# omerbt/TokenFlow

Hardware: NVIDIA H100
Metric: frames/sec for 40-frame 512x512 SD1.5 50-step edit (higher is better)
Workload: dtype fp16

## Files before the change

tokenflow_b200/_build.py:

```python
from __future__ import annotations

import hashlib
import os
import shutil
import subprocess
import sys
from pathlib import Path

PKG_DIR = Path(__file__).resolve().parent
CSRC = PKG_DIR / "csrc"
LIB_PATH = PKG_DIR / "libtokenflow_b200.so"
STAMP = PKG_DIR / ".libtokenflow_b200.stamp"

SOURCES = ["tf_capi.cu", "tf_unit_rows.cu", "tf_propagate.cu", "tf_nn_field.cu", "tf_ext_attn.cu", "tf_cfg_ddim.cu",
           "tf_comm.cu", "tf_body.cu", "tf_pixels.cu", "tf_resize.cu",
           "tf_canny.cu"]
HEADERS = ["tf_common.cuh", "tf_kernels.h", "tf_wgmma.cuh", "../../include/tokenflow_b200.h",
           "../../include/tokenflow_b200_vpred.h"]

NVCC_FLAGS = [
    "-gencode", "arch=compute_90a,code=sm_90a",
    "-O3", "-std=c++17", "-lineinfo",
    "-Xcompiler", "-fPIC",
    "-Xcompiler", "-ffp-contract=off",
    "-Xptxas", "-v",
    "--expt-relaxed-constexpr",
    "-cudart", "static",
]


def _nvcc() -> str:
    for cand in (os.environ.get("NVCC"), shutil.which("nvcc"), "/usr/local/cuda/bin/nvcc"):
        if cand and os.path.exists(cand):
            return cand
    raise RuntimeError("nvcc not found (set NVCC=/path/to/nvcc)")


def _digest() -> str:
    h = hashlib.sha256()
    for name in SOURCES + HEADERS:
        h.update((CSRC / name).read_bytes())
    h.update(" ".join(NVCC_FLAGS).encode())
    return h.hexdigest()


def needs_build() -> bool:
    return not (LIB_PATH.exists() and STAMP.exists() and STAMP.read_text().strip() == _digest())


def build(force: bool = False, verbose: bool = False) -> Path:
    if not force and not needs_build():
# ... 33 lines not shown
```

tokenflow_b200/csrc/tf_body.cu:

```cuda
#include "tf_common.cuh"
#include "tf_kernels.h"

namespace tf {
namespace {

constexpr int kGnMaxThreads = 512;
static_assert(kGnMaxChannels / 8 <= kGnMaxThreads, "one row of 8-channel columns must fit in a CTA");
constexpr int kGnStatsChunkBytes = 64 << 10;
constexpr int kGnApplyChunkBytes = 128 << 10;
constexpr int kGnUnroll = 4;

struct GnLayout {
  int cols, rows, threads;
  long long stats_px, apply_px;
  int stats_chunks, apply_chunks;
};

GnLayout gn_layout(long long hw, int c) {
  GnLayout L;
  L.cols = c / 8;
  L.rows = kGnMaxThreads / L.cols > 0 ? kGnMaxThreads / L.cols : 1;
  L.threads = (L.cols * L.rows + 31) / 32 * 32;
  auto chunk = [&](int bytes) {
    long long px = bytes / (2LL * c);
    px = (px + L.rows - 1) / L.rows * L.rows;
    return px < L.rows ? (long long)L.rows : px;
  };
  L.stats_px = chunk(kGnStatsChunkBytes);
  L.apply_px = chunk(kGnApplyChunkBytes);
  L.stats_chunks = (int)((hw + L.stats_px - 1) / L.stats_px);
  L.apply_chunks = (int)((hw + L.apply_px - 1) / L.apply_px);
  return L;
}

constexpr int kGnG4ApplyChunksPerSample = 64;

GnLayout gn_layout_g4(long long hw, int c) {
  GnLayout L = gn_layout(hw, c);
  long long px = (hw + kGnG4ApplyChunksPerSample - 1) / kGnG4ApplyChunksPerSample;
  px = (px + L.rows - 1) / L.rows * L.rows;
  if (px > L.apply_px) {
    L.apply_px = px;
    L.apply_chunks = (int)((hw + px - 1) / px);
  }
  return L;
}

__device__ __forceinline__ void unpack8(const uint4& raw, float (&v)[8]) {
  const __half2* h = reinterpret_cast<const __half2*>(&raw);
#pragma unroll
  for (int e = 0; e < 4; ++e) {
    const float2 f = __half22float2(h[e]);
    v[2 * e] = f.x;
    v[2 * e + 1] = f.y;
  }
}

__device__ __forceinline__ float round_h(float x) { return __half2float(__float2half_rn(x)); }

template <bool kBias>
__device__ __forceinline__ float group_shift(const __half* xn, const __half* bias_n, int g, int cpg) {
  const int c = g * cpg;
  const float v = __half2float(xn[c]);
  return kBias ? round_h(v + __half2float(bias_n[c])) : v;
}

template <bool kBias, int kCpg>
__global__ void __launch_bounds__(kGnMaxThreads, 2)
gn_stats_kernel(const __half* __restrict__ x, const __half* __restrict__ bias, long long bias_stride, long long hw,
                int C, int cpg_rt, int G, int rows, long long chunk_px, int chunks, double2* __restrict__ ws) {
  const int cpg = kCpg ? kCpg : cpg_rt;
  extern __shared__ double2 part[];
  const int cols = C >> 3;
  const int tid = threadIdx.x;
  const int row = tid / cols, col = tid - row * cols;
  const int n = blockIdx.y, chunk = blockIdx.x;
  const __half* xn = x + (long long)n * hw * C;
  const __half* bias_n = kBias ? bias + (long long)n * bias_stride : nullptr;
  if (row < rows) {
    const int c0 = col * 8;
    float bv[8], shift[8];
    if (kBias) unpack8(*reinterpret_cast<const uint4*>(bias_n + c0), bv);
#pragma unroll
    for (int e = 0; e < 8; ++e) shift[e] = group_shift<kBias>(xn, bias_n, (c0 + e) / cpg, cpg);
    const int g_lo = c0 / cpg;
    int hi_mask = 0;
#pragma unroll
    for (int e = 0; e < 8; ++e) hi_mask |= ((c0 + e) / cpg != g_lo) << e;
    double2 lo = make_double2(0.0, 0.0), hi = make_double2(0.0, 0.0);
    const long long p_begin = (long long)chunk * chunk_px;
    const long long p_end = p_begin + chunk_px < hw ? p_begin + chunk_px : hw;
// ... 114 lines not shown
  for (long long p = p_begin + row; p < p_end; p += (long long)rows * kUnroll) {
    uint4 raw[kUnroll];
#pragma unroll
    for (int u = 0; u < kUnroll; ++u) {
      const long long q = p + (long long)u * rows;
      if (q < p_end) raw[u] = *reinterpret_cast<const uint4*>(xn + q * C + c0);
    }
#pragma unroll
    for (int u = 0; u < kUnroll; ++u) {
      const long long q = p + (long long)u * rows;
      if (q < p_end) {
        float v[8];
        unpack8(raw[u], v);
        uint4 w;
        __half2* h = reinterpret_cast<__half2*>(&w);
#pragma unroll
        for (int e = 0; e < 4; ++e) {
          float y[2];
#pragma unroll
          for (int k = 0; k < 2; ++k) {
            const int i = 2 * e + k;
            const float xv = kBias ? round_h(v[i] + bv[i]) : v[i];
            y[k] = round_h(fmaf(a[i], xv, b[i]));
            if (kSilu) y[k] = y[k] / (1.0f + expf(-y[k]));
          }
          h[e] = __floats2half2_rn(y[0], y[1]);
        }
        *reinterpret_cast<uint4*>(on + q * C + c0) = w;
      }
    }
  }
}

__device__ __forceinline__ float gelu_erf(float v) {
  constexpr float kAlpha = 0.70710678118654752440f;
  return v * 0.5f * (1.0f + erff(v * kAlpha));
}

__device__ __forceinline__ float geglu1(float xv, float gv) { return xv * round_h(gelu_erf(gv)); }

__global__ void __launch_bounds__(256)
geglu_kernel(const __half* __restrict__ xh, const __half* __restrict__ gate, long long n_vec, long long n,
             __half* __restrict__ out) {
  const long long stride = (long long)gridDim.x * blockDim.x;
  for (long long i = (long long)blockIdx.x * blockDim.x + threadIdx.x; i < n_vec; i += stride) {
    float xv[8], gv[8];
    unpack8(reinterpret_cast<const uint4*>(xh)[i], xv);
    unpack8(reinterpret_cast<const uint4*>(gate)[i], gv);
    uint4 w;
    __half2* h = reinterpret_cast<__half2*>(&w);
#pragma unroll
    for (int e = 0; e < 4; ++e) h[e] = __floats2half2_rn(geglu1(xv[2 * e], gv[2 * e]), geglu1(xv[2 * e + 1], gv[2 * e + 1]));
    reinterpret_cast<uint4*>(out)[i] = w;
  }
  if (blockIdx.x == 0 && threadIdx.x == 0) {
    for (long long j = n_vec * 8; j < n; ++j)
      out[j] = __float2half_rn(geglu1(__half2float(xh[j]), __half2float(gate[j])));
  }
}

}

long long group_norm_nhwc_workspace(long long n, long long hw, int c, int groups) {
  if (n <= 0 || hw <= 0 || c <= 0 || (c & 7) || groups <= 0 || c % groups) return 0;
  return n * groups * (long long)gn_layout(hw, c).stats_chunks * (long long)sizeof(double2);
}

namespace {

template <int kCpg>
int launch_gn(const GnLayout& L, const __half* xp, const __half* bp, long long bias_stride, const __half* gp,
              const __half* btp, long long n, long long hw, int c, int groups, float eps, int silu, double2* ws,
              __half* op, cudaStream_t stream, const char* stats_what, const char* apply_what) {
// ... 67 lines not shown
```

tokenflow_b200/csrc/tf_capi.cu:

```cuda
#include <algorithm>
#include <atomic>
#include <cmath>
#include <cstdarg>
#include <cstdio>
#include <cstring>
#include <vector>

#include "../../include/tokenflow_b200.h"
#include "../../include/tokenflow_b200_vpred.h"
#include "tf_common.cuh"
#include "tf_kernels.h"

namespace tf {

static thread_local char g_err[512] = "";
static std::atomic<long long> g_launches{0};

void set_last_error(const char* fmt, ...) {
  va_list ap;
  va_start(ap, fmt);
  vsnprintf(g_err, sizeof(g_err), fmt, ap);
  va_end(ap);
}

int check_cuda(cudaError_t e, const char* what) {
  if (e == cudaSuccess) return TF_OK;
  set_last_error("%s: %s (%s)", what, cudaGetErrorName(e), cudaGetErrorString(e));
  return TF_ERR_CUDA;
}

int sm_count() {
  static int cached[64] = {0};
  int dev = 0;
  if (cudaGetDevice(&dev) != cudaSuccess || dev < 0 || dev >= 64) return 132;
  if (cached[dev] == 0) {
    int n = 0;
    if (cudaDeviceGetAttribute(&n, cudaDevAttrMultiProcessorCount, dev) != cudaSuccess || n <= 0) n = 132;
    cached[dev] = n;
  }
  return cached[dev];
}

// ... 322 lines not shown
  if (!canny_sizes_ok(n, h, w, "tf_canny_u8")) return TF_ERR_INVALID_ARGUMENT;
  if (!(low == low) || !(high == high)) {
    set_last_error("tf_canny_u8: NaN threshold");
    return TF_ERR_INVALID_ARGUMENT;
  }
  if (low > high) std::swap(low, high);
  const double lo = std::floor(low), hi = std::floor(high);
  const int ilo = (int)std::min(std::max(lo, -1.0), 2040.0), ihi = (int)std::min(std::max(hi, -1.0), 2040.0);
  if (n == 0) return TF_OK;
  const long long need = canny_workspace(n, h, w);
  if (workspace_bytes < need) {
    set_last_error("tf_canny_u8: workspace of %lld bytes, %lld needed", (long long)workspace_bytes, need);
    return TF_ERR_INVALID_ARGUMENT;
  }
  if (!frames || !workspace || (!edges_u8 && !cond_f16) || !aligned16(workspace) ||
      (cond_f16 && (reinterpret_cast<uintptr_t>(cond_f16) & 1u))) {
    set_last_error("tf_canny_u8: NULL or misaligned pointer (frames, a 16-byte aligned workspace, and at least one "
                   "output are needed)");
    return TF_ERR_INVALID_ARGUMENT;
  }
  int e = launch_canny(frames, n, h, w, ilo, ihi, workspace, edges_u8, cond_f16, static_cast<cudaStream_t>(stream));
  if (!e) g_launches += 5;
  return e;
}

int tf_geglu(const void* xh, const void* gate, int64_t n, void* out, tf_stream_t stream) {
  if (n < 0) { set_last_error("tf_geglu: n=%lld", (long long)n); return TF_ERR_INVALID_ARGUMENT; }
  if (n == 0) return TF_OK;
  if (!xh || !gate || !out || !aligned16(xh) || !aligned16(gate) || !aligned16(out)) {
    set_last_error("tf_geglu: NULL or misaligned pointer");
    return TF_ERR_INVALID_ARGUMENT;
  }
  int e = launch_geglu(xh, gate, n, out, static_cast<cudaStream_t>(stream));
  if (!e) g_launches += 1;
  return e;
}

int tf_nn_field(const void* x_unit, const void* piv_unit, const int32_t* kf_a, const int32_t* kf_b, int F, int S,
                int dim, int K, int32_t* idx_a, int32_t* idx_b, tf_stream_t stream) {
  if (F < 0 || S < 0 || dim <= 0 || (dim & 7) || K <= 0) {
    set_last_error("tf_nn_field: bad shape F=%d S=%d dim=%d K=%d", F, S, dim, K);
    return TF_ERR_INVALID_ARGUMENT;
  }
  if (F > 0 && !kf_a) { set_last_error("tf_nn_field: kf_a is NULL"); return TF_ERR_INVALID_ARGUMENT; }
  for (int f0 = 0; f0 < F; f0 += kMaxFrames) {
    FrameTable tab;
    const int fc = F - f0 < kMaxFrames ? F - f0 : kMaxFrames;
    if (int e = fill_table(tab, kf_a + f0, kf_b ? kf_b + f0 : nullptr, nullptr, fc, K, "tf_nn_field")) return e;
  }
  if (F == 0 || S == 0) return TF_OK;
  bool need_b = false;
  if (kf_b) for (int f = 0; f < F; ++f) need_b |= kf_b[f] >= 0;
  if (!x_unit || !piv_unit || !idx_a || (need_b && !idx_b) || !aligned16(x_unit) || !aligned16(piv_unit)) {
    set_last_error("tf_nn_field: NULL or misaligned pointer");
    return TF_ERR_INVALID_ARGUMENT;
  }
  const __half* xu = static_cast<const __half*>(x_unit);
  for (int f0 = 0; f0 < F; f0 += kMaxFrames) {
    FrameTable tab;
    const int fc = F - f0 < kMaxFrames ? F - f0 : kMaxFrames;
    fill_table(tab, kf_a + f0, kf_b ? kf_b + f0 : nullptr, nullptr, fc, K, "tf_nn_field");
    const long long off = (long long)f0 * S;
    int e = launch_nn_field(xu + off * dim, piv_unit, tab, fc, S, dim, K, idx_a + off, idx_b ? idx_b + off : nullptr,
                            static_cast<cudaStream_t>(stream));
    if (e) return e;
    g_launches += 1;
// ... 166 lines not shown
```

tokenflow_b200/csrc/tf_common.cuh:

```cuda
#pragma once

#include <cuda.h>
#include <cuda_fp16.h>
#include <cuda_runtime.h>
#include <stdint.h>
#include <stdio.h>

namespace tf {

void set_last_error(const char* fmt, ...);
int  check_cuda(cudaError_t e, const char* what);

enum Status : int {
  TF_OK = 0,
  TF_ERR_INVALID_ARGUMENT = 1,
  TF_ERR_CUDA = 2,
  TF_ERR_UNSUPPORTED = 3,
  TF_ERR_DRIVER = 4,
};

CUresult encode_tiled(CUtensorMap* map, CUtensorMapDataType dtype, uint32_t rank, const void* base,
                      const uint64_t* dims, const uint64_t* strides_bytes ,
                      const uint32_t* box, CUtensorMapSwizzle swizzle);

// ... 19 lines not shown
               : "memory");
}
__device__ __forceinline__ bool mbar_try_wait(uint64_t* bar, uint32_t parity) {
  uint32_t ok;
  asm volatile(
      "{\n\t.reg .pred p;\n\t"
      "mbarrier.try_wait.parity.shared::cta.b64 p, [%1], %2;\n\t"
      "selp.u32 %0, 1, 0, p;\n\t}\n"
      : "=r"(ok)
      : "r"(smem_u32(bar)), "r"(parity)
      : "memory");
  return ok != 0;
}
__device__ __forceinline__ uint64_t global_timer_ns() {
  uint64_t t;
  asm volatile("mov.u64 %0, %%globaltimer;" : "=l"(t));
  return t;
}
__device__ __forceinline__ void mbar_wait(uint64_t* bar, uint32_t parity) {
  uint32_t spins = 0;
  uint64_t t0 = 0;
  while (!mbar_try_wait(bar, parity)) {
    if ((++spins & 2047u) == 0) {
      const uint64_t now = global_timer_ns();
      if (t0 == 0) t0 = now;
      if (now - t0 > 2000000000ull) __trap();
    }
  }
}

__device__ __forceinline__ void tma_prefetch_desc(const CUtensorMap* m) {
  asm volatile("prefetch.tensormap [%0];" ::"l"(reinterpret_cast<uint64_t>(m)) : "memory");
}
__device__ __forceinline__ void tma_load_3d(void* smem_dst, const CUtensorMap* m, uint64_t* bar, int c0,
                                            int c1, int c2) {
  asm volatile(
      "cp.async.bulk.tensor.3d.shared::cluster.global.tile.mbarrier::complete_tx::bytes"
      " [%0], [%1, {%3, %4, %5}], [%2];"
      ::"r"(smem_u32(smem_dst)), "l"(reinterpret_cast<uint64_t>(m)), "r"(smem_u32(bar)), "r"(c0), "r"(c1),
      "r"(c2)
      : "memory");
}
__device__ __forceinline__ void tma_load_4d(void* smem_dst, const CUtensorMap* m, uint64_t* bar, int c0,
                                            int c1, int c2, int c3) {
  asm volatile(
      "cp.async.bulk.tensor.4d.shared::cluster.global.tile.mbarrier::complete_tx::bytes"
      " [%0], [%1, {%3, %4, %5, %6}], [%2];"
      ::"r"(smem_u32(smem_dst)), "l"(reinterpret_cast<uint64_t>(m)), "r"(smem_u32(bar)), "r"(c0), "r"(c1),
      "r"(c2), "r"(c3)
      : "memory");
}

__device__ __forceinline__ uint64_t wgmma_desc(uint32_t smem_addr, uint32_t lbo_bytes, uint32_t sbo_bytes) {
  uint64_t d = 0;
  d |= static_cast<uint64_t>((smem_addr & 0x3FFFFu) >> 4);
  d |= static_cast<uint64_t>((lbo_bytes >> 4) & 0x3FFFu) << 16;
  d |= static_cast<uint64_t>((sbo_bytes >> 4) & 0x3FFFu) << 32;
  d |= static_cast<uint64_t>(1) << 62;
  return d;
}
__device__ __forceinline__ void wgmma_fence() { asm volatile("wgmma.fence.sync.aligned;" ::: "memory"); }
__device__ __forceinline__ void wgmma_commit() { asm volatile("wgmma.commit_group.sync.aligned;" ::: "memory"); }
template <int kPending>
__device__ __forceinline__ void wgmma_wait() {
  asm volatile("wgmma.wait_group.sync.aligned %0;" ::"n"(kPending) : "memory");
}
template <int N>
__device__ __forceinline__ void reg_fence(float (&r)[N]) {
#pragma unroll
  for (int i = 0; i < N; ++i) asm volatile("" : "+f"(r[i])::"memory");
}

__device__ __forceinline__ uint32_t pack_f16x2_rn(float lo, float hi) {
  uint32_t r;
  asm("cvt.rn.f16x2.f32 %0, %1, %2;" : "=r"(r) : "f"(hi), "f"(lo));
  return r;
}
__device__ __forceinline__ float fast_exp2(float x) {
  float y;
  asm("ex2.approx.ftz.f32 %0, %1;" : "=f"(y) : "f"(x));
  return y;
}
#endif

}
```

tokenflow_b200/csrc/tf_kernels.h:

```cpp
#pragma once

#include <cuda_runtime.h>
#include <stdint.h>

namespace tf {

constexpr int kMaxFrames = 64;
struct FrameTable {
  int32_t kf_a[kMaxFrames];
  int32_t kf_b[kMaxFrames];
  float w[kMaxFrames];
};

int launch_unit_rows(const void* x, int x_is_f32, long long rows, int dim, long long row_stride, void* out_f16,
                     cudaStream_t stream);

int launch_layernorm_unit_rows(const void* x_f16, long long rows, int dim, long long row_stride, const float* gamma,
                               const float* beta, float eps, void* out_f16, cudaStream_t stream);

int launch_layernorm_rows(const void* x_f16, long long rows, int dim, long long row_stride, const float* gamma,
                          const float* beta, float eps, void* y_out, long long y_row_stride, void* unit_out,
                          long long unit_row_stride, long long unit_rows, cudaStream_t stream);

int launch_cfg_ddim(const void* eps_uncond, const void* eps_cond, const void* x, const float* coef_dev, float guidance,
                    long long n, void* out, cudaStream_t stream);
int launch_ddim(const void* eps, const void* x, const float* coef_dev, long long n, void* out, cudaStream_t stream);
int launch_cfg_ddim_v(const void* v_uncond, const void* v_cond, const void* x, const float* coef_dev, float guidance,
                      long long n, void* out, cudaStream_t stream);
int launch_ddim_v(const void* v, const void* x, const float* coef_dev, long long n, void* out, cudaStream_t stream);

constexpr int kGnMaxChannels = 4096;
long long group_norm_nhwc_workspace(long long n, long long hw, int c, int groups);
int launch_group_norm_nhwc(const void* x, const void* bias, long long bias_stride, const void* gamma, const void* beta,
                           long long n, long long hw, int c, int groups, float eps, int silu, void* workspace,
                           void* out, cudaStream_t stream);
int launch_geglu(const void* xh, const void* gate, long long n, void* out, cudaStream_t stream);

int launch_frames_to_nhwc(const void* frames, long long n, void* out, cudaStream_t stream);
int launch_nhwc_to_frames(const void* x, long long n, void* frames, cudaStream_t stream);

int resize_taps(int in, int out);
void resize_coeffs(int in, int out, int32_t* bounds, int32_t* coeffs);
int launch_resize_h(const void* in, long long n_rows, int w_in, int w, const int32_t* bounds, const int32_t* coeffs,
                    int taps, void* out, cudaStream_t stream);
int launch_resize_v(const void* in, long long n, int h_in, int h, int w, const int32_t* bounds, const int32_t* coeffs,
                    int taps, void* out, cudaStream_t stream);

long long canny_workspace(long long n, int h, int w);
int launch_canny(const void* frames, long long n, int h, int w, int low, int high, void* workspace, void* edges,
                 void* cond, cudaStream_t stream);

int launch_propagate(const void* A, const int32_t* idx_a, const int32_t* idx_b, const FrameTable& tab, int F,
                     int S, int dim, int K, const void* residual, void* out, int out_is_f32, long long F_total,
                     cudaStream_t stream);

int launch_nn_field(const void* x_unit, const void* piv_unit, const FrameTable& tab, int F, int S, int dim,
                    int K, int32_t* idx_a, int32_t* idx_b, cudaStream_t stream);

struct AttnSample {
  int32_t out_sample;
  int32_t q_sample;
  int32_t k_sample0;
  int32_t v_sample0;
  int32_t n_kv;
};
constexpr int kMaxAttnSamples = 160;
struct AttnTable {
  AttnSample s[kMaxAttnSamples];
};
// ... 25 lines not shown
```

tokenflow_b200/csrc/tf_pixels.cu:

```cuda
#include "tf_common.cuh"
#include "tf_kernels.h"

namespace tf {
namespace {

__device__ __forceinline__ float round_h(float x) { return __half2float(__float2half_rn(x)); }

__device__ __forceinline__ __half byte_to_input(unsigned v) {
  const float unit = round_h(__fdiv_rn((float)v, 255.0f));
  return __float2half_rn(round_h(2.0f * unit) - 1.0f);
}

__device__ __forceinline__ unsigned char output_to_byte(float x) {
  float y = round_h(round_h(x * 0.5f) + 0.5f);
  if (isnan(y)) return 0;
  y = fminf(fmaxf(y, 0.0f), 1.0f);
  return (unsigned char)round_h(y * 255.0f);
}

__global__ void __launch_bounds__(256) frames_to_input_kernel(const uint8_t* __restrict__ in, long long n_vec,
                                                              long long n, __half* __restrict__ out) {
  const long long stride = (long long)gridDim.x * blockDim.x;
  for (long long i = (long long)blockIdx.x * blockDim.x + threadIdx.x; i < n_vec; i += stride) {
    const uint2 raw = reinterpret_cast<const uint2*>(in)[i];
    uint4 w;
    __half* h = reinterpret_cast<__half*>(&w);
#pragma unroll
    for (int e = 0; e < 8; ++e) h[e] = byte_to_input(((e < 4 ? raw.x : raw.y) >> (8 * (e & 3))) & 0xffu);
    reinterpret_cast<uint4*>(out)[i] = w;
  }
  if (blockIdx.x == 0)
    for (long long j = n_vec * 8 + threadIdx.x; j < n; j += blockDim.x) out[j] = byte_to_input(in[j]);
}

__global__ void __launch_bounds__(256) output_to_frames_kernel(const __half* __restrict__ in, long long n_vec,
                                                               long long n, uint8_t* __restrict__ out) {
  const long long stride = (long long)gridDim.x * blockDim.x;
  for (long long i = (long long)blockIdx.x * blockDim.x + threadIdx.x; i < n_vec; i += stride) {
    const uint4 raw = reinterpret_cast<const uint4*>(in)[i];
// ... 38 lines not shown
```

tokenflow_b200/ops.py:

```python
from __future__ import annotations

import ctypes
from pathlib import Path
from typing import Optional, Sequence, Tuple

import torch

LIB_NAME = "libtokenflow_b200.so"
TF_MAX_FRAMES = 64
TF_MAX_ATTN_SAMPLES = 160
TF_COMM_ID_BYTES = 128

_c_i32p = ctypes.POINTER(ctypes.c_int32)
_c_f32p = ctypes.POINTER(ctypes.c_float)

_SIGNATURES = {
    "tf_version": (ctypes.c_int, []),
    "tf_last_error": (ctypes.c_char_p, []),
    "tf_launch_count": (ctypes.c_int64, []),
    "tf_unit_rows": (ctypes.c_int, [ctypes.c_void_p, ctypes.c_int, ctypes.c_int64, ctypes.c_int, ctypes.c_int64,
                                    ctypes.c_void_p, ctypes.c_void_p]),
    "tf_layernorm_unit_rows": (ctypes.c_int, [ctypes.c_void_p, ctypes.c_int64, ctypes.c_int, ctypes.c_int64,
                                              ctypes.c_void_p, ctypes.c_void_p, ctypes.c_float, ctypes.c_void_p,
                                              ctypes.c_void_p]),
# ... 16 lines not shown
                                    ctypes.c_void_p, ctypes.c_int, ctypes.c_void_p]),
    "tf_ext_attn_fwd": (ctypes.c_int, [ctypes.c_void_p, ctypes.c_void_p, ctypes.c_void_p, ctypes.c_int64,
                                       ctypes.c_int, ctypes.c_int, ctypes.c_int, ctypes.c_int, ctypes.c_float,
                                       ctypes.c_int, ctypes.c_void_p, ctypes.c_void_p]),
    "tf_ext_attn_fwd_rows": (ctypes.c_int, [ctypes.c_void_p, ctypes.c_int, ctypes.c_int64, ctypes.c_void_p,
                                            ctypes.c_void_p, ctypes.c_int, ctypes.c_int64, ctypes.c_int, _c_i32p,
                                            _c_i32p, _c_i32p, _c_i32p, _c_i32p, ctypes.c_int, ctypes.c_int,
                                            ctypes.c_int, ctypes.c_float, ctypes.c_int, ctypes.c_int, ctypes.c_void_p,
                                            ctypes.c_void_p]),
    "tf_group_norm_nhwc_workspace": (ctypes.c_int64, [ctypes.c_int64, ctypes.c_int64, ctypes.c_int, ctypes.c_int]),
    "tf_group_norm_nhwc": (ctypes.c_int, [ctypes.c_void_p, ctypes.c_void_p, ctypes.c_int64, ctypes.c_void_p,
                                          ctypes.c_void_p, ctypes.c_int64, ctypes.c_int64, ctypes.c_int, ctypes.c_int,
                                          ctypes.c_float, ctypes.c_int, ctypes.c_void_p, ctypes.c_int64,
                                          ctypes.c_void_p, ctypes.c_void_p]),
    "tf_frames_to_nhwc": (ctypes.c_int, [ctypes.c_void_p, ctypes.c_int64, ctypes.c_void_p, ctypes.c_void_p]),
    "tf_nhwc_to_frames": (ctypes.c_int, [ctypes.c_void_p, ctypes.c_int64, ctypes.c_void_p, ctypes.c_void_p]),
    "tf_resize_taps": (ctypes.c_int, [ctypes.c_int, ctypes.c_int]),
    "tf_resize_coeffs": (ctypes.c_int, [ctypes.c_int, ctypes.c_int, ctypes.c_void_p, ctypes.c_void_p]),
    "tf_resize_u8": (ctypes.c_int, [ctypes.c_void_p, ctypes.c_int64, ctypes.c_int, ctypes.c_int, ctypes.c_int,
                                    ctypes.c_int, ctypes.c_void_p, ctypes.c_void_p, ctypes.c_int, ctypes.c_void_p,
                                    ctypes.c_void_p, ctypes.c_int, ctypes.c_void_p, ctypes.c_void_p, ctypes.c_void_p]),
    "tf_canny_workspace": (ctypes.c_int64, [ctypes.c_int64, ctypes.c_int, ctypes.c_int]),
    "tf_canny_u8": (ctypes.c_int, [ctypes.c_void_p, ctypes.c_int64, ctypes.c_int, ctypes.c_int, ctypes.c_double,
                                   ctypes.c_double, ctypes.c_void_p, ctypes.c_int64, ctypes.c_void_p, ctypes.c_void_p,
                                   ctypes.c_void_p]),
    "tf_geglu": (ctypes.c_int, [ctypes.c_void_p, ctypes.c_void_p, ctypes.c_int64, ctypes.c_void_p, ctypes.c_void_p]),
}

_VPRED_SIGNATURES = {
    "tf_cfg_ddim_v": _SIGNATURES["tf_cfg_ddim"],
    "tf_ddim_v": _SIGNATURES["tf_ddim"],
}


class TokenflowB200Error(RuntimeError):
    pass


def library_path() -> Path:
    return Path(__file__).resolve().parent / LIB_NAME


_LIB = None


def load_library() -> ctypes.CDLL:
    global _LIB
    if _LIB is not None:
        return _LIB
    path = library_path()
    if not path.exists():
        raise TokenflowB200Error(
            f"{path} is missing: build it with `python -m tokenflow_b200._build` "
            "(or __graft_entry__.build()).  tokenflow_b200 has no fallback path.")
    lib = ctypes.CDLL(str(path))
    for name, (res, args) in list(_SIGNATURES.items()) + list(_VPRED_SIGNATURES.items()):
        fn = getattr(lib, name)
        fn.restype = res
        fn.argtypes = args
    _LIB = lib
    return lib


def exported_symbols() -> Sequence[str]:
    return tuple(_SIGNATURES.keys())


def blend_weights(n_frames: int) -> Sequence[float]:
    f = torch.arange(0, n_frames)
    d1 = torch.abs(f - n_frames // 2)
    d2 = torch.abs(f + n_frames - n_frames // 2)
    return torch.sigmoid(d2 / (d1 + d2)).tolist()


def propagate_bytes(F_: int, S: int, dim: int, kf_a, kf_b, with_residual: bool, out_esz: int = 2) -> float:
    kfs = {int(a) for a in kf_a} | {int(b) for b in kf_b if int(b) >= 0}
    n_idx = F_ + sum(1 for b in kf_b if int(b) >= 0)
    return (3.0 * F_ * S * dim * out_esz + (3.0 * F_ * S * dim * 2 if with_residual else 0.0)
            + 3.0 * len(kfs) * S * dim * 2 + 4.0 * S * n_idx)


def _dense(t: torch.Tensor, memory_format=torch.contiguous_format) -> torch.Tensor:
    if t.is_contiguous(memory_format=memory_format) and t.data_ptr() % 16 == 0:
        return t
    return t.clone(memory_format=memory_format)


def _i32(vals: Sequence[int]):
    return (ctypes.c_int32 * len(vals))(*[int(v) for v in vals])
# ... 364 lines not shown
        assert frames.dtype == torch.uint8 and frames.dim() == 4 and frames.shape[-1] == 3 and frames.is_cuda
        assert edges or cond
        frames = frames.contiguous()
        n, h, w, _ = frames.shape
        dev = frames.device
        ws_bytes = int(self.lib.tf_canny_workspace(n, h, w))
        if ws_bytes < 0:
            self._check(1, "tf_canny_workspace")
        ws = torch.empty(max(ws_bytes, 16), dtype=torch.uint8, device=dev)
        e = c = None
        if edges:
            e = out_edges if out_edges is not None else torch.empty((n, h, w), dtype=torch.uint8, device=dev)
            assert e.shape == (n, h, w) and e.dtype == torch.uint8 and e.is_contiguous()
        if cond:
            c = out_cond if out_cond is not None else torch.empty((n, 3, h, w), dtype=torch.float16, device=dev,
                                                                  memory_format=torch.channels_last)
            assert c.shape == (n, 3, h, w) and c.dtype == torch.float16 and c.is_contiguous(memory_format=torch.channels_last)
        work = 3.0 * n * h * w + (n * h * w if edges else 0) + (6.0 * n * h * w if cond else 0)
        ptr = lambda t: t.data_ptr() if t is not None else None
        self._timed("tf_canny_u8", work, lambda: self._check(self.lib.tf_canny_u8(
            frames.data_ptr(), n, h, w, float(low), float(high), ws.data_ptr(), ws.numel(), ptr(e), ptr(c),
            self._stream()), "tf_canny_u8"))
        return e, c

    def geglu(self, xh: torch.Tensor, gate: torch.Tensor) -> torch.Tensor:
        assert xh.dtype == gate.dtype == torch.float16 and xh.shape == gate.shape
        xh, gate = _dense(xh), _dense(gate)
        out = torch.empty_like(xh)
        n = xh.numel()
        self._timed("tf_geglu", 3.0 * n * 2, lambda: self._check(
            self.lib.tf_geglu(xh.data_ptr(), gate.data_ptr(), n, out.data_ptr(), self._stream()), "tf_geglu"))
        return out


_DEFAULT_OPS = None


def default_ops() -> CudaOps:
    global _DEFAULT_OPS
    if _DEFAULT_OPS is None:
        _DEFAULT_OPS = CudaOps()
    return _DEFAULT_OPS


_BODY_OPS = False


def body_ops() -> Optional[CudaOps]:
    global _BODY_OPS
    if _BODY_OPS is False:
        try:
            _BODY_OPS = default_ops()
        except TokenflowB200Error:
            _BODY_OPS = None
    return _BODY_OPS


def all_gather(t: torch.Tensor, world_size: int, group=None, comm=None) -> torch.Tensor:
    if world_size == 1:
        return t
    if comm is not None and t.is_cuda:
        return comm.all_gather(t)
    import torch.distributed as dist
    t = t.contiguous()
    out = torch.empty((world_size * t.shape[0],) + tuple(t.shape[1:]), dtype=t.dtype, device=t.device)
    dist.all_gather_into_tensor(out, t, group=group)
# ... 42 lines not shown
```

tokenflow_b200/sd_unet.py:

```python
from __future__ import annotations

import math
from dataclasses import dataclass
from typing import Optional, Tuple

import torch
import torch.nn as nn
import torch.nn.functional as F


@dataclass
class UNetConfig:
    in_channels: int = 4
    out_channels: int = 4
    block_out_channels: Tuple[int, ...] = (320, 640, 1280, 1280)
    layers_per_block: int = 2
    cross_attention_dim: int = 768
    num_heads: Tuple[int, ...] = (8, 8, 8, 8)
    norm_num_groups: int = 32
    use_linear_projection: bool = False
    sample_size: int = 64


def sd15_config() -> UNetConfig:
# ... 58 lines not shown
        ctx = cross_attention_dim if cross_attention_dim is not None else query_dim
        self.to_q = nn.Linear(query_dim, inner, bias=False)
        self.to_k = nn.Linear(ctx, inner, bias=False)
        self.to_v = nn.Linear(ctx, inner, bias=False)
        self.to_out = nn.ModuleList([nn.Linear(inner, query_dim), nn.Dropout(0.0)])

    def head_to_batch_dim(self, t: torch.Tensor) -> torch.Tensor:
        b, s, _ = t.shape
        h = self.heads
        return t.reshape(b, s, h, -1).permute(0, 2, 1, 3).reshape(b * h, s, -1)

    def batch_to_head_dim(self, t: torch.Tensor) -> torch.Tensor:
        bh, s, d = t.shape
        h = self.heads
        return t.reshape(bh // h, h, s, d).permute(0, 2, 1, 3).reshape(bh // h, s, d * h)

    def forward(self, hidden_states, encoder_hidden_states=None, attention_mask=None):
        ctx = hidden_states if encoder_hidden_states is None else encoder_hidden_states
        b, s, _ = hidden_states.shape
        h = self.heads
        q = self.to_q(hidden_states).view(b, s, h, -1).transpose(1, 2)
        k = self.to_k(ctx).view(b, ctx.shape[1], h, -1).transpose(1, 2)
        v = self.to_v(ctx).view(b, ctx.shape[1], h, -1).transpose(1, 2)
        o = F.scaled_dot_product_attention(q, k, v, attn_mask=attention_mask, scale=self.scale)
        o = o.transpose(1, 2).reshape(b, s, -1)
        return self.to_out[1](self.to_out[0](o))


class GEGLU(nn.Module):
    def __init__(self, dim_in: int, dim_out: int):
        super().__init__()
        self.proj = nn.Linear(dim_in, dim_out * 2)

    def forward(self, x):
        w_x, w_g = self.proj.weight.chunk(2, dim=0)
        b_x, b_g = self.proj.bias.chunk(2, dim=0)
        xh, g = F.linear(x, w_x, b_x), F.linear(x, w_g, b_g)
        if xh.is_cuda and xh.dtype == g.dtype == torch.float16:
            from .ops import body_ops
            ops = body_ops()
            if ops is not None:
                return ops.geglu(xh, g)
        return xh * F.gelu(g)


class FeedForward(nn.Module):
    def __init__(self, dim: int, mult: int = 4):
        super().__init__()
        self.net = nn.ModuleList([GEGLU(dim, dim * mult), nn.Dropout(0.0), nn.Linear(dim * mult, dim)])

    def forward(self, x):
        for m in self.net:
            x = m(x)
        return x


class BasicTransformerBlock(nn.Module):

    def __init__(self, dim: int, heads: int, dim_head: int, cross_attention_dim: int):
        super().__init__()
        self.only_cross_attention = False
        self.use_ada_layer_norm = False
        self.use_ada_layer_norm_zero = False
        self.norm1 = nn.LayerNorm(dim)
        self.attn1 = Attention(dim, None, heads, dim_head)
        self.norm2 = BodyLayerNorm(dim)
        self.attn2 = Attention(dim, cross_attention_dim, heads, dim_head)
# ... 297 lines not shown
```

Measured before the change: 2.881.

## Fuse GEGLU projection GEMM with bias and gelu gating into one WGMMA kernel

Adds a persistent warp-specialized Hopper GEMM (TMA loads, 4-stage mbarrier pipeline, two consumer warpgroups, WGMMA) that computes both the value and gate halves of the GEGLU projection per tile. It applies bias, gelu and gating in the epilogue and TMA-stores the result. This replaces two separate cuBLAS linears plus an elementwise geglu kernel, removing the round trip of two large intermediate activations through HBM. The trade-off is a hand-written GEMM with a fixed 256x64 tile that may be slower than cuBLAS on the matmul itself, and it keeps an fp16 rounding order meant to match the unfused path.

```diff
diff --git a/include/tokenflow_b200_gemm.h b/include/tokenflow_b200_gemm.h
--- /dev/null
+++ b/include/tokenflow_b200_gemm.h
@@ -0,0 +1,18 @@
+#ifndef TOKENFLOW_B200_GEMM_H_
+#define TOKENFLOW_B200_GEMM_H_
+
+#include <stdint.h>
+
+#include "tokenflow_b200.h"
+
+#ifdef __cplusplus
+extern "C" {
+#endif
+
+int tf_geglu_gemm(const void* x, const void* w, const void* bias, int64_t M, int K, int inner, void* out,
+                  tf_stream_t stream);
+
+#ifdef __cplusplus
+}
+#endif
+#endif
diff --git a/tokenflow_b200/_build.py b/tokenflow_b200/_build.py
--- a/tokenflow_b200/_build.py
+++ b/tokenflow_b200/_build.py
@@ -14,9 +14,9 @@
 
 SOURCES = ["tf_capi.cu", "tf_unit_rows.cu", "tf_propagate.cu", "tf_nn_field.cu", "tf_ext_attn.cu", "tf_cfg_ddim.cu",
            "tf_comm.cu", "tf_body.cu", "tf_pixels.cu", "tf_resize.cu",
-           "tf_canny.cu"]
+           "tf_canny.cu", "tf_geglu_gemm.cu"]
 HEADERS = ["tf_common.cuh", "tf_kernels.h", "tf_wgmma.cuh", "../../include/tokenflow_b200.h",
-           "../../include/tokenflow_b200_vpred.h"]
+           "../../include/tokenflow_b200_vpred.h", "../../include/tokenflow_b200_gemm.h"]
 
 NVCC_FLAGS = [
     "-gencode", "arch=compute_90a,code=sm_90a",
diff --git a/tokenflow_b200/csrc/tf_body.cu b/tokenflow_b200/csrc/tf_body.cu
--- a/tokenflow_b200/csrc/tf_body.cu
+++ b/tokenflow_b200/csrc/tf_body.cu
@@ -55,8 +55,6 @@
     v[2 * e + 1] = f.y;
   }
 }
-
-__device__ __forceinline__ float round_h(float x) { return __half2float(__float2half_rn(x)); }
 
 template <bool kBias>
 __device__ __forceinline__ float group_shift(const __half* xn, const __half* bias_n, int g, int cpg) {
@@ -237,13 +235,6 @@
   }
 }
 
-__device__ __forceinline__ float gelu_erf(float v) {
-  constexpr float kAlpha = 0.70710678118654752440f;
-  return v * 0.5f * (1.0f + erff(v * kAlpha));
-}
-
-__device__ __forceinline__ float geglu1(float xv, float gv) { return xv * round_h(gelu_erf(gv)); }
-
 __global__ void __launch_bounds__(256)
 geglu_kernel(const __half* __restrict__ xh, const __half* __restrict__ gate, long long n_vec, long long n,
              __half* __restrict__ out) {
diff --git a/tokenflow_b200/csrc/tf_capi.cu b/tokenflow_b200/csrc/tf_capi.cu
--- a/tokenflow_b200/csrc/tf_capi.cu
+++ b/tokenflow_b200/csrc/tf_capi.cu
@@ -8,6 +8,7 @@
 
 #include "../../include/tokenflow_b200.h"
 #include "../../include/tokenflow_b200_vpred.h"
+#include "../../include/tokenflow_b200_gemm.h"
 #include "tf_common.cuh"
 #include "tf_kernels.h"
 
@@ -396,6 +397,23 @@
     return TF_ERR_INVALID_ARGUMENT;
   }
   int e = launch_geglu(xh, gate, n, out, static_cast<cudaStream_t>(stream));
+  if (!e) g_launches += 1;
+  return e;
+}
+
+int tf_geglu_gemm(const void* x, const void* w, const void* bias, int64_t M, int K, int inner, void* out,
+                  tf_stream_t stream) {
+  if (M < 0 || M >= INT32_MAX - 128 || K <= 0 || (K & 7) || inner <= 0 || (inner & 7)) {
+    set_last_error("tf_geglu_gemm: bad shape M=%lld K=%d inner=%d (K %% 8 == 0, inner %% 8 == 0, M < 2^31 - 128)",
+                   (long long)M, K, inner);
+    return TF_ERR_INVALID_ARGUMENT;
+  }
+  if (M == 0) return TF_OK;
+  if (!x || !w || !bias || !out || !aligned16(x) || !aligned16(w) || !aligned16(bias) || !aligned16(out)) {
+    set_last_error("tf_geglu_gemm: NULL or misaligned pointer");
+    return TF_ERR_INVALID_ARGUMENT;
+  }
+  int e = launch_geglu_gemm(x, w, bias, M, K, inner, out, static_cast<cudaStream_t>(stream));
   if (!e) g_launches += 1;
   return e;
 }
diff --git a/tokenflow_b200/csrc/tf_common.cuh b/tokenflow_b200/csrc/tf_common.cuh
--- a/tokenflow_b200/csrc/tf_common.cuh
+++ b/tokenflow_b200/csrc/tf_common.cuh
@@ -75,6 +75,13 @@
 __device__ __forceinline__ void tma_prefetch_desc(const CUtensorMap* m) {
   asm volatile("prefetch.tensormap [%0];" ::"l"(reinterpret_cast<uint64_t>(m)) : "memory");
 }
+__device__ __forceinline__ void tma_load_2d(void* smem_dst, const CUtensorMap* m, uint64_t* bar, int c0, int c1) {
+  asm volatile(
+      "cp.async.bulk.tensor.2d.shared::cluster.global.tile.mbarrier::complete_tx::bytes"
+      " [%0], [%1, {%3, %4}], [%2];"
+      ::"r"(smem_u32(smem_dst)), "l"(reinterpret_cast<uint64_t>(m)), "r"(smem_u32(bar)), "r"(c0), "r"(c1)
+      : "memory");
+}
 __device__ __forceinline__ void tma_load_3d(void* smem_dst, const CUtensorMap* m, uint64_t* bar, int c0,
                                             int c1, int c2) {
   asm volatile(
@@ -93,6 +100,19 @@
       "r"(c2), "r"(c3)
       : "memory");
 }
+
+__device__ __forceinline__ void tma_store_2d(const CUtensorMap* m, const void* smem_src, int c0, int c1) {
+  asm volatile("cp.async.bulk.tensor.2d.global.shared::cta.bulk_group [%0, {%2, %3}], [%1];"
+               ::"l"(reinterpret_cast<uint64_t>(m)), "r"(smem_u32(smem_src)), "r"(c0), "r"(c1)
+               : "memory");
+}
+__device__ __forceinline__ void tma_store_commit() { asm volatile("cp.async.bulk.commit_group;" ::: "memory"); }
+__device__ __forceinline__ void tma_store_wait_read() { asm volatile("cp.async.bulk.wait_group.read 0;" ::: "memory"); }
+__device__ __forceinline__ void tma_store_wait_all() { asm volatile("cp.async.bulk.wait_group 0;" ::: "memory"); }
+__device__ __forceinline__ void fence_proxy_async_smem() {
+  asm volatile("fence.proxy.async.shared::cta;" ::: "memory");
+}
+__device__ __forceinline__ void wg_bar_sync(int id) { asm volatile("bar.sync %0, 128;" ::"r"(id) : "memory"); }
 
 __device__ __forceinline__ uint64_t wgmma_desc(uint32_t smem_addr, uint32_t lbo_bytes, uint32_t sbo_bytes) {
   uint64_t d = 0;
@@ -124,6 +144,13 @@
   asm("ex2.approx.ftz.f32 %0, %1;" : "=f"(y) : "f"(x));
   return y;
 }
+__device__ __forceinline__ float round_h(float x) { return __half2float(__float2half_rn(x)); }
+
+__device__ __forceinline__ float gelu_erf(float v) {
+  constexpr float kAlpha = 0.70710678118654752440f;
+  return v * 0.5f * (1.0f + erff(v * kAlpha));
+}
+__device__ __forceinline__ float geglu1(float xv, float gv) { return xv * round_h(gelu_erf(gv)); }
 #endif
 
 }
diff --git a/tokenflow_b200/csrc/tf_geglu_gemm.cu b/tokenflow_b200/csrc/tf_geglu_gemm.cu
--- /dev/null
+++ b/tokenflow_b200/csrc/tf_geglu_gemm.cu
@@ -0,0 +1,188 @@
+#include "tf_common.cuh"
+#include "tf_kernels.h"
+#include "tf_wgmma.cuh"
+
+namespace tf {
+namespace {
+
+constexpr int kConsumers = 2;
+constexpr int kBlockM = 128 * kConsumers;
+constexpr int kBlockN = 64;
+constexpr int kChunkK = 64;
+constexpr int kStages = 4;
+constexpr int kThreads = 128 * kConsumers + 32;
+constexpr int kABytes = kBlockM * 128;
+constexpr int kBHalfBytes = kBlockN * 128;
+constexpr int kStageBytes = kABytes + 2 * kBHalfBytes;
+constexpr int kOutBytes = 128 * kBlockN * 2;
+constexpr size_t kSmemBytes =
+    1024 + (size_t)kStages * kStageBytes + (size_t)kConsumers * kOutBytes + 2 * kStages * sizeof(uint64_t);
+
+__device__ __forceinline__ void stage_half(const float (&acc)[64], const __half* __restrict__ bias, int n0, int inner,
+                                           int r0, int col0, uint8_t* tile) {
+#pragma unroll
+  for (int jb = 0; jb < 8; ++jb) {
+    const int col = n0 + col0 + 8 * jb;
+    float2 bx = make_float2(0.f, 0.f), bg = make_float2(0.f, 0.f);
+    if (col < inner) {
+      bx = __half22float2(*reinterpret_cast<const __half2*>(bias + col));
+      bg = __half22float2(*reinterpret_cast<const __half2*>(bias + inner + col));
+    }
+#pragma unroll
+    for (int r = 0; r < 2; ++r) {
+      const int row = r0 + 8 * r;
+      const float x0 = round_h(acc[4 * jb + 2 * r] + bx.x);
+      const float x1 = round_h(acc[4 * jb + 2 * r + 1] + bx.y);
+      const float g0 = round_h(acc[4 * (jb + 8) + 2 * r] + bg.x);
+      const float g1 = round_h(acc[4 * (jb + 8) + 2 * r + 1] + bg.y);
+      *reinterpret_cast<__half2*>(tile + row * 128 + ((jb ^ (row & 7)) << 4) + col0 * 2) =
+          __floats2half2_rn(geglu1(x0, g0), geglu1(x1, g1));
+    }
+  }
+}
+
+__global__ void __launch_bounds__(kThreads, 1)
+geglu_gemm_kernel(const __grid_constant__ CUtensorMap map_x, const __grid_constant__ CUtensorMap map_w,
+                  const __grid_constant__ CUtensorMap map_out, const __half* __restrict__ bias, int inner,
+                  int n_col_tiles, long long n_tiles, int n_k) {
+  extern __shared__ uint8_t smem_raw[];
+  uint8_t* smem = reinterpret_cast<uint8_t*>((reinterpret_cast<uintptr_t>(smem_raw) + 1023) & ~uintptr_t(1023));
+  uint8_t* out_tiles = smem + kStages * kStageBytes;
+  uint64_t* full = reinterpret_cast<uint64_t*>(out_tiles + kConsumers * kOutBytes);
+  uint64_t* empty = full + kStages;
+
+  if (threadIdx.x == 0) {
+    tma_prefetch_desc(&map_x);
+    tma_prefetch_desc(&map_w);
+    tma_prefetch_desc(&map_out);
+    for (int i = 0; i < kStages; ++i) {
+      mbar_init(&full[i], 1);
+      mbar_init(&empty[i], 4 * kConsumers);
+    }
+    fence_mbar_init();
+  }
+  __syncthreads();
+
+  if (threadIdx.x >= 128 * kConsumers) {
+    if (threadIdx.x == 128 * kConsumers) {
+      int st = 0;
+      uint32_t ph = 0;
+      bool refill = false;
+      for (long long t = blockIdx.x; t < n_tiles; t += gridDim.x) {
+        const int m0 = (int)(t / n_col_tiles) * kBlockM;
+        const int n0 = (int)(t % n_col_tiles) * kBlockN;
+        for (int kc = 0; kc < n_k; ++kc) {
+          if (refill) mbar_wait(&empty[st], ph ^ 1u);
+          uint8_t* dst = smem + st * kStageBytes;
+          mbar_arrive_expect_tx(&full[st], (uint32_t)kStageBytes);
+          tma_load_2d(dst, &map_x, &full[st], kc * kChunkK, m0);
+          tma_load_3d(dst + kABytes, &map_w, &full[st], kc * kChunkK, n0, 0);
+          tma_load_3d(dst + kABytes + kBHalfBytes, &map_w, &full[st], kc * kChunkK, n0, 1);
+          if (++st == kStages) { st = 0; ph ^= 1u; refill = true; }
+        }
+      }
+    }
+    return;
+  }
+
+  const int wg = threadIdx.x >> 7;
+  const int warp = (threadIdx.x >> 5) & 3;
+  const int lane = threadIdx.x & 31;
+  const uint32_t ring = smem_u32(smem);
+  auto release = [&](int s) {
+    __syncwarp();
+    if (lane == 0) mbar_arrive(&empty[s]);
+  };
+  int st = 0, prev = 0;
+  uint32_t ph = 0;
+  for (long long t = blockIdx.x; t < n_tiles; t += gridDim.x) {
+    float acc0[64], acc1[64];
+#pragma unroll
+    for (int i = 0; i < 64; ++i) acc0[i] = acc1[i] = 0.0f;
+    for (int kc = 0; kc < n_k; ++kc) {
+      mbar_wait(&full[st], ph);
+      __syncwarp();
+      const uint32_t b = ring + st * kStageBytes + kABytes;
+      const uint32_t a = ring + st * kStageBytes + wg * 128 * 128;
+      wgmma_fence();
+#pragma unroll
+      for (int k4 = 0; k4 < kChunkK / 16; ++k4) {
+        const uint64_t db = wgmma_desc(b + k4 * 32, 16, 1024);
+        wgmma_ss<128>(acc0, wgmma_desc(a + k4 * 32, 16, 1024), db, 1u);
+        wgmma_ss<128>(acc1, wgmma_desc(a + 64 * 128 + k4 * 32, 16, 1024), db, 1u);
+      }
+      wgmma_commit();
+      if (kc > 0) {
+        wgmma_wait<1>();
+        release(prev);
+      }
+      prev = st;
+      if (++st == kStages) { st = 0; ph ^= 1u; }
+    }
+    wgmma_wait<0>();
+    reg_fence(acc0);
+    reg_fence(acc1);
+    release(prev);
+
+    const int m0 = (int)(t / n_col_tiles) * kBlockM + 128 * wg;
+    const int n0 = (int)(t % n_col_tiles) * kBlockN;
+    uint8_t* tile = out_tiles + wg * kOutBytes;
+    const bool issuer = (threadIdx.x & 127) == 0;
+    if (issuer) tma_store_wait_read();
+    wg_bar_sync(1 + wg);
+    const int r0 = 16 * warp + (lane >> 2);
+    stage_half(acc0, bias, n0, inner, r0, 2 * (lane & 3), tile);
+    stage_half(acc1, bias, n0, inner, r0 + 64, 2 * (lane & 3), tile);
+    fence_proxy_async_smem();
+    wg_bar_sync(1 + wg);
+    if (issuer) {
+      tma_store_2d(&map_out, tile, n0, m0);
+      tma_store_commit();
+    }
+  }
+  if ((threadIdx.x & 127) == 0) tma_store_wait_all();
+}
+
+}
+
+int launch_geglu_gemm(const void* x, const void* w, const void* bias, long long M, int K, int inner, void* out,
+                      cudaStream_t stream) {
+  if (M == 0) return TF_OK;
+  const int n_col_tiles = (inner + kBlockN - 1) / kBlockN;
+  const long long n_tiles = (M + kBlockM - 1) / kBlockM * n_col_tiles;
+  const int n_k = (K + kChunkK - 1) / kChunkK;
+  CUtensorMap map_x, map_w, map_out;
+  {
+    const uint64_t dims[2] = {(uint64_t)K, (uint64_t)M};
+    const uint64_t strides[1] = {(uint64_t)K * 2};
+    const uint32_t box[2] = {(uint32_t)kChunkK, (uint32_t)kBlockM};
+    CUresult r = encode_tiled(&map_x, CU_TENSOR_MAP_DATA_TYPE_FLOAT16, 2, x, dims, strides, box,
+                              CU_TENSOR_MAP_SWIZZLE_128B);
+    if (r != CUDA_SUCCESS) { set_last_error("tf_geglu_gemm: cuTensorMapEncodeTiled(x) failed: %d", (int)r); return TF_ERR_DRIVER; }
+  }
+  {
+    const uint64_t dims[3] = {(uint64_t)K, (uint64_t)inner, 2};
+    const uint64_t strides[2] = {(uint64_t)K * 2, (uint64_t)inner * K * 2};
+    const uint32_t box[3] = {(uint32_t)kChunkK, (uint32_t)kBlockN, 1};
+    CUresult r = encode_tiled(&map_w, CU_TENSOR_MAP_DATA_TYPE_FLOAT16, 3, w, dims, strides, box,
+                              CU_TENSOR_MAP_SWIZZLE_128B);
+    if (r != CUDA_SUCCESS) { set_last_error("tf_geglu_gemm: cuTensorMapEncodeTiled(w) failed: %d", (int)r); return TF_ERR_DRIVER; }
+  }
+  {
+    const uint64_t dims[2] = {(uint64_t)inner, (uint64_t)M};
+    const uint64_t strides[1] = {(uint64_t)inner * 2};
+    const uint32_t box[2] = {(uint32_t)kBlockN, 128};
+    CUresult r = encode_tiled(&map_out, CU_TENSOR_MAP_DATA_TYPE_FLOAT16, 2, out, dims, strides, box,
+                              CU_TENSOR_MAP_SWIZZLE_128B);
+    if (r != CUDA_SUCCESS) { set_last_error("tf_geglu_gemm: cuTensorMapEncodeTiled(out) failed: %d", (int)r); return TF_ERR_DRIVER; }
+  }
+  if (check_cuda(cudaFuncSetAttribute(geglu_gemm_kernel, cudaFuncAttributeMaxDynamicSharedMemorySize, (int)kSmemBytes),
+                 "tf_geglu_gemm smem attribute"))
+    return TF_ERR_CUDA;
+  const long long grid = n_tiles < (long long)sm_count() ? n_tiles : (long long)sm_count();
+  geglu_gemm_kernel<<<(unsigned)grid, kThreads, kSmemBytes, stream>>>(
+      map_x, map_w, map_out, static_cast<const __half*>(bias), inner, n_col_tiles, n_tiles, n_k);
+  return check_cuda(cudaGetLastError(), "tf_geglu_gemm launch");
+}
+
+}
diff --git a/tokenflow_b200/csrc/tf_kernels.h b/tokenflow_b200/csrc/tf_kernels.h
--- a/tokenflow_b200/csrc/tf_kernels.h
+++ b/tokenflow_b200/csrc/tf_kernels.h
@@ -35,6 +35,8 @@
                            long long n, long long hw, int c, int groups, float eps, int silu, void* workspace,
                            void* out, cudaStream_t stream);
 int launch_geglu(const void* xh, const void* gate, long long n, void* out, cudaStream_t stream);
+int launch_geglu_gemm(const void* x, const void* w, const void* bias, long long M, int K, int inner, void* out,
+                      cudaStream_t stream);
 
 int launch_frames_to_nhwc(const void* frames, long long n, void* out, cudaStream_t stream);
 int launch_nhwc_to_frames(const void* x, long long n, void* frames, cudaStream_t stream);
diff --git a/tokenflow_b200/csrc/tf_pixels.cu b/tokenflow_b200/csrc/tf_pixels.cu
--- a/tokenflow_b200/csrc/tf_pixels.cu
+++ b/tokenflow_b200/csrc/tf_pixels.cu
@@ -3,8 +3,6 @@
 
 namespace tf {
 namespace {
-
-__device__ __forceinline__ float round_h(float x) { return __half2float(__float2half_rn(x)); }
 
 __device__ __forceinline__ __half byte_to_input(unsigned v) {
   const float unit = round_h(__fdiv_rn((float)v, 255.0f));
diff --git a/tokenflow_b200/ops.py b/tokenflow_b200/ops.py
--- a/tokenflow_b200/ops.py
+++ b/tokenflow_b200/ops.py
@@ -72,6 +72,11 @@
     "tf_ddim_v": _SIGNATURES["tf_ddim"],
 }
 
+_GEMM_SIGNATURES = {
+    "tf_geglu_gemm": (ctypes.c_int, [ctypes.c_void_p, ctypes.c_void_p, ctypes.c_void_p, ctypes.c_int64, ctypes.c_int,
+                                     ctypes.c_int, ctypes.c_void_p, ctypes.c_void_p]),
+}
+
 
 class TokenflowB200Error(RuntimeError):
     pass
@@ -94,7 +99,8 @@
             f"{path} is missing: build it with `python -m tokenflow_b200._build` "
             "(or __graft_entry__.build()).  tokenflow_b200 has no fallback path.")
     lib = ctypes.CDLL(str(path))
-    for name, (res, args) in list(_SIGNATURES.items()) + list(_VPRED_SIGNATURES.items()):
+    for name, (res, args) in (list(_SIGNATURES.items()) + list(_VPRED_SIGNATURES.items())
+                              + list(_GEMM_SIGNATURES.items())):
         fn = getattr(lib, name)
         fn.restype = res
         fn.argtypes = args
@@ -525,6 +531,31 @@
             self.lib.tf_geglu(xh.data_ptr(), gate.data_ptr(), n, out.data_ptr(), self._stream()), "tf_geglu"))
         return out
 
+    @staticmethod
+    def geglu_proj_supported(x: torch.Tensor, weight: torch.Tensor, bias: Optional[torch.Tensor]) -> bool:
+        if bias is None or not (x.is_cuda and x.dtype == weight.dtype == bias.dtype == torch.float16):
+            return False
+        K = x.shape[-1]
+        if x.dim() < 2 or weight.dim() != 2 or weight.shape[1] != K or weight.shape[0] % 2 or bias.shape != weight.shape[:1]:
+            return False
+        inner = weight.shape[0] // 2
+        return K % 8 == 0 and inner % 8 == 0 and inner > 0 \
+            and x.numel() // K < 2 ** 31 - 128 \
+            and weight.device == bias.device == x.device
+
+    def geglu_proj(self, x: torch.Tensor, weight: torch.Tensor, bias: torch.Tensor) -> torch.Tensor:
+        K = x.shape[-1]
+        inner = weight.shape[0] // 2
+        x2 = _dense(x.reshape(-1, K))
+        w, b = _dense(weight), _dense(bias)
+        M = x2.shape[0]
+        out = torch.empty((M, inner), dtype=torch.float16, device=x.device)
+        nbytes = 2.0 * (M * K + 2 * inner * K + 2 * inner + M * inner)
+        self._timed("tf_geglu", nbytes, lambda: self._check(
+            self.lib.tf_geglu_gemm(x2.data_ptr(), w.data_ptr(), b.data_ptr(), M, K, inner, out.data_ptr(),
+                                   self._stream()), "tf_geglu_gemm"))
+        return out.view(*x.shape[:-1], inner)
+
 
 _DEFAULT_OPS = None
 
diff --git a/tokenflow_b200/sd_unet.py b/tokenflow_b200/sd_unet.py
--- a/tokenflow_b200/sd_unet.py
+++ b/tokenflow_b200/sd_unet.py
@@ -114,7 +114,26 @@
         super().__init__()
         self.proj = nn.Linear(dim_in, dim_out * 2)
 
-    def forward(self, x):
+    def _half_params(self):
+        w, b = self.proj.weight, self.proj.bias
+        key = (w.data_ptr(), w._version, b.data_ptr(), b._version)
+        cache = self.__dict__.get("_tf_half_params")
+        if cache is None or cache[0] != key:
+            cache = (key, w.detach().half().contiguous(), b.detach().half().contiguous())
+            self.__dict__["_tf_half_params"] = cache
+        return cache[1], cache[2]
+
+    def forward(self, x):
+        w, b = self.proj.weight, self.proj.bias
+        if x.is_cuda and x.dtype == torch.float16 and b is not None:
+            if w.dtype != torch.float16 and torch.is_autocast_enabled("cuda") \
+                    and torch.get_autocast_dtype("cuda") == torch.float16:
+                w, b = self._half_params()
+            from .ops import CudaOps, body_ops
+            if CudaOps.geglu_proj_supported(x, w, b):
+                ops = body_ops()
+                if ops is not None:
+                    return ops.geglu_proj(x, w, b)
         w_x, w_g = self.proj.weight.chunk(2, dim=0)
         b_x, b_g = self.proj.bias.chunk(2, dim=0)
         xh, g = F.linear(x, w_x, b_x), F.linear(x, w_g, b_g)
```

Measured after the change: 2.934, median of 6. 1.8% higher.
